# salesforce/warp-drive

Measured on AMD Instinct MI355X. Metric: env steps/sec, TagContinuous 5 taggers x 100 runners, higher is better.
Workload: dtype f32; 1 GPU; BASELINE configs[2]: TagContinuous 5 taggers x 100 runners, partial obs K=10 (F=71), num_envs=2000 per GPU; tick = sample_actions (2 heads) + step + reset of finished replicas (one fused launch); num_envs_per_gpu=2000, num_agents=105, launch_mode=plan, kernels_per_tick=1, ticks_per_launch=1, parallelism=env-replica sharding x1

## Files before the change

warp_drive_amd/csrc/kernels/tc_fast.h:

```cpp
#pragma once
#include "wd_common.h"
#include "tc_fetch.h"
#include "tc_sample.h"
#include "tc_move.h"
#include "tc_tags.h"
#include "tc_reset.h"
#include "tc_knn.h"
#include "tc_rows.h"

namespace {

template <int KMAX, bool FUSED, bool EXACTK, int IDB, bool SAMPLE = FUSED, bool LOOP = false, int SN = 0, int SA = 0,
          int ST = 0>
__device__ __forceinline__ int tc_fast_impl(const TcArgs &a, const TcFuse &fz, unsigned char *smem, int n_acc,
                                            int n_turn, int tick = 0, int n_taggers_in = 0, TcCarry *cy = nullptr,
                                            const TcLoopConsts *lc = nullptr) {
  WD_TC_PROBE_TICK(LOOP, tick);
  const int N = a.N, K = EXACTK ? KMAX : a.K;
  const int F = 7 * K + 1;
  int tid_ = threadIdx.x;
  if constexpr (LOOP) asm volatile("" : "+v"(tid_));
  const int tid = tid_, T_ = WD_TC_BLOCKDIM;
  const int epb = max(1, T_ / N);
  const int n_waves = (T_ + 63) >> 6, wave = __builtin_amdgcn_readfirstlane(tid >> 6), lane = tid & 63;
  const size_t slab_acc_bytes = tc_align16((size_t)4 * epb * N * n_acc);
  const bool compact = (epb == 1);
  const size_t slab_turn_bytes = tc_align16((size_t)4 * epb * N * n_turn);
  const bool one_slab = tc_one_slab(N);
  const TcFastLds l = tc_carve_fast(smem, epb, N, K, n_waves,
                                    !SAMPLE ? 0 : one_slab ? max(slab_acc_bytes, slab_turn_bytes) : slab_acc_bytes + slab_turn_bytes,
                                    compact);
  const TcTables &tb = l.tb;
  float *const slab_acc = (float *)smem, *const slab_turn = (float *)(smem + (one_slab ? 0 : slab_acc_bytes));
  float *const stage = l.stage + (size_t)wave * l.stage_dwords;
  const int el = tid / N, ag = tid - el * N;
  const float invK = 1.0f / (float)K, invN = 1.0f / (float)N;
  const int NP = ((N + 3) & ~3) + 8;

  int group = blockIdx.x;
#ifndef WD_TC_BLOCK_ORDER_PLAIN
  if constexpr (IDB == 7) {
    const int bx = blockIdx.x & 7, bq = gridDim.x >> 3, br = gridDim.x & 7;
    group = bx * bq + min(bx, br) + (int)(blockIdx.x >> 3);
  }
#endif
  const int env0 = a.env_begin + group * epb;
  __builtin_amdgcn_s_setprio(3);
  WD_TC_PROBE_RT(16); WD_TC_PROBE(0); WD_TC_PROBE_HW(21);
  TcIn in;
  bool reloaded = false;
  if constexpr (LOOP) {
    in = cy->in;
    reloaded = cy->reload != 0;
    if (reloaded) {
      tc_load_state(in, a, fz, env0, epb, N, n_acc, n_turn, tid, tick == 0);
      cy->in.type = in.type; cy->in.skill = in.skill; cy->in.step_reward = in.step_reward;
    }
  } else {
    tc_issue_loads<FUSED, SAMPLE>(in, a, fz, env0, epb, N, n_acc, n_turn, tid, slab_acc, slab_turn, true);
  }
  const bool tab_in_lds = (n_acc <= WD_TC_TAB) && (n_turn <= WD_TC_TAB);
  int n_taggers_ = n_taggers_in;
  if constexpr (LOOP) {
    if (tick == 0) n_taggers_ = tc_build_tables(tb, a, N, n_acc, n_turn, tab_in_lds, in);
  } else {
    n_taggers_ = tc_build_tables(tb, a, N, n_acc, n_turn, tab_in_lds, in);
  }
  const int n_taggers = n_taggers_;
  if (env0 >= a.E) return n_taggers;
  if constexpr (!LOOP) WD_TC_PROBE(1);

  const int env = env0 + el;
  const bool active = (el < epb) && (env < a.E);
  const int gi = env * N + ag;
  const int li = tid;
  const int agents_here = min(epb, a.E - env0) * N;
  if constexpr (LOOP) {
    if (active && ag == 0) a.done[env] = 0;
    static_assert(!LOOP || (SN > 0 && SA > 0 && ST == WD_TC_BLOCKDIM), "the multi-tick entry is built for one shape");
    tc_fetch_slabs_straight<SN, SA, ST>(slab_acc, slab_turn, fz.probs_acc, fz.probs_turn, env0, wave, lane);
    WD_TC_PROBE(1);
  }
  int2 sampled = in.sampled;
  const unsigned long long live_mask = __ballot(active && in.sg != 0);
  if constexpr (!LOOP) {
    if (compact && lane == 0) tb.live_cnt[wave] = __popcll(live_mask);
  }
  if constexpr ((IDB != 7) && (KMAX <= 12)) {
    if (compact && tid < 64) tb.cell_cnt[tid] = 0;
  }
  if constexpr (LOOP) {
    static_assert(!LOOP || IDB == 7, "tc_sample_heads_carried samples from two slabs: replicas of at most 128 agents");
    sampled = tc_sample_heads_carried<SA>(fz, in.epoch, cy->k0, cy->k1, active, gi, li, slab_acc, slab_turn, n_acc, n_turn);
    if (compact && lane == 0) tb.live_cnt[wave] = __popcll(live_mask);
  } else if (FUSED) {
    if (active && ag == 0) a.done[env] = 0;
    if (SAMPLE) sampled = tc_sample_heads(a, fz, in, active, gi, li, slab_acc, slab_turn, n_acc, n_turn, env0, epb);
  }
  WD_TC_PROBE(2);
  __syncthreads();
  WD_TC_PROBE(3);
  int my_c = ag, n_live = N;
  if (compact) {
    int before = 0;
    n_live = 0;
    for (int w2 = 0; w2 < n_waves; ++w2) {
      const int c = tb.live_cnt[w2];
      before += (w2 < wave) ? c : 0;
      n_live += c;
    }
    my_c = before + __popcll(live_mask & ((1ull << lane) - 1ull));
  }
  constexpr bool PRE = (IDB != 7) && (KMAX <= 12);
  constexpr bool TIE_TABLE = (IDB != 7);
  bool pre_on = false;
  int cells_C = 0;
  float cell_len = 0.0f, cell_inv = 0.0f;
  int my_cell = 0, my_cell_slot = 0;
  uint4 hint_a = make_uint4(~0u, ~0u, ~0u, ~0u), hint_b = hint_a;
  if constexpr (PRE) {
    pre_on = compact && (a.knn_prev != nullptr) && (n_live >= WD_TC_PRE_MIN_LIVE) && (l.stage_dwords >= WD_TC_LIST_DWORDS);
    if (pre_on && active && in.sg != 0) {
      const uint4 *const h = (const uint4 *)(a.knn_prev + (size_t)(env * N + ag) * 8);
      hint_a = h[0];
      hint_b = h[1];
    }
    if (pre_on) {
      cells_C = tc_cell_grid(n_live, K);
      cell_len = a.grid_length / (float)max(cells_C, 1);
      cell_inv = (float)cells_C / a.grid_length;
    }
  }

  float edge_pen = 0.0f, my_x = 0.0f, my_y = 0.0f;
  const int sg = in.sg;
  const bool is_runner = active && (in.type == 0) && (sg != 0);
  if (active) {
    const TcMoved m = tc_move<LOOP>(a, tb, in, sampled, gi, tab_in_lds, LOOP ? cy : nullptr, LOOP ? lc : nullptr);
    edge_pen = m.edge_pen; my_x = m.x; my_y = m.y;
    if constexpr (LOOP) {
      cy->in.x = m.x; cy->in.y = m.y;
      cy->in.cleared = (sg == 0) ? 1 : 0;
    }
    l.xy[el * NP + ag] = make_float2(sg ? m.x : (PRE && pre_on ? __builtin_nanf("") : WD_BIG), m.y);
    if (compact) {
      if (sg) {
        bool by_cell = false;
        if constexpr (PRE) {
          if (cells_C != 0) {
            const int2 c = tc_cell_xy(m.x, m.y, cell_inv, cells_C);
            my_cell = tc_cell_place(c, cells_C);
            my_cell_slot = atomicAdd(&tb.cell_cnt[my_cell], 1);
            by_cell = true;
          }
        }
        if (!by_cell) {
          l.xyc[my_c] = make_float2(m.x, m.y);
          l.cid[1 + my_c] = (short)ag;
          if (PRE && pre_on) {
            uint4 *const slot = (uint4 *)(l.stage + (size_t)(my_c >> 6) * l.stage_dwords) + 2 * (my_c & 63);
            slot[0] = hint_a;
            slot[1] = hint_b;
          }
        }
      }
      if (ag == 0) {
        l.cid[0] = -1;
        if (PRE && pre_on) {
          l.xyc[n_live] = make_float2(WD_BIG, WD_BIG);
          l.xy[N] = make_float2(__builtin_nanf(""), 0.0f);
        }
      }
    }
    tc_feat_store(l.feat, li, m.ft);
    l.sig[li] = (sg ? 1 : 0) | (in.cleared ? 2 : 0);
    if ((in.cleared != 0) != (sg == 0)) a.obs_rows_cleared[gi] = sg ? 0 : 1;
    l.tagcnt[li] = 0;
    if (ag == 0) {
      const int t = in.tstep + 1;
      a.timestep[env] = t;
      tb.tstep[el] = t;
      if constexpr (LOOP) tb.tfrac[el] = (float)tc_div_const((double)t, (double)a.T, lc->r_T);
      else tb.tfrac[el] = (float)((double)t / (double)a.T);
      if constexpr (LOOP) {
        cy->in.tstep = t;
        if (reloaded) tb.nrun[el] = in.nrun;
      } else {
        tb.nrun[el] = in.nrun;
      }
    }
  }
  WD_TC_PROBE(4);
  __syncthreads();
  WD_TC_PROBE(5);
  int cell_incl = 0;
  if constexpr (PRE) {
    if (cells_C != 0) {
      const int cnt = tb.cell_cnt[lane];
      cell_incl = cnt;
#pragma unroll
      for (int d = 1; d < 64; d <<= 1) {
        const int up = __shfl_up(cell_incl, d, 64);
        cell_incl += (lane >= d) ? up : 0;
      }
      my_c = __builtin_amdgcn_ds_bpermute(my_cell << 2, cell_incl - cnt) + my_cell_slot;
      if (active && sg != 0) {
        l.xyc[my_c] = make_float2(my_x, my_y);
        l.cid[1 + my_c] = (short)ag;
        uint4 *const slot = (uint4 *)(l.stage + (size_t)(my_c >> 6) * l.stage_dwords) + 2 * (my_c & 63);
        slot[0] = hint_a;
        slot[1] = hint_b;
      }
    }
  }

  bool tagged = false;
  if constexpr (LOOP) {
    if (is_runner)
      tagged = tc_find_tag<true>(a, tb, l.xy + el * NP, l.tagcnt + el * N, &tb.nrun[el], n_taggers, my_x, my_y, lc->Bc);
  } else {
    if (is_runner)
      tagged = tc_find_tag(a, tb, l.xy + el * NP, l.tagcnt + el * N, &tb.nrun[el], n_taggers, my_x, my_y);
  }
  if constexpr (PRE) {
    if (cells_C != 0) __syncthreads();
  }

  WD_TC_PROBE(6);
  int nid[KMAX + 1], rank[KMAX + 1];
#pragma unroll
  for (int k = 0; k <= KMAX; ++k) { nid[k] = -1; rank[k] = k; }
  bool in_order = true;
  __builtin_amdgcn_s_setprio(2);
  const bool searcher = compact ? (tid < n_live) : (active && sg != 0);
  const float2 *const sxy = compact ? l.xyc : l.xy + el * NP;
  const int n_cand = compact ? n_live : N;
  int row_agent = ag;
  constexpr int L = KMAX + ((EXACTK && IDB == 7) ? 2 : 3);
  const bool split = compact && (n_waves == 2) && (n_live <= 64) && (n_live >= 16) &&
                     (l.stage_dwords >= 64 * L);
  const int j_half = split ? (((n_live + 7) >> 3) << 2) : n_cand;
  const bool helper = split && (wave == 1);
  unsigned S[L];
  bool prefiltered = false;
  unsigned extra = 0xffffffffu;
  if constexpr (PRE) {
    if (pre_on) {
      unsigned Tb = 0u;
      float sx = 0.0f, sy = 0.0f;
      int2 scell = make_int2(0, 0);
      if (searcher) {
        const uint4 *const slot = (const uint4 *)stage + 2 * lane;
        const uint4 pa = slot[0], pb = slot[1];
        sx = sxy[ag].x; sy = sxy[ag].y;
        Tb = tc_knn_bound16<KMAX>(l.xy, N, sx, sy, pa, pb, K);
        if (cells_C != 0) {
          scell = tc_cell_xy(sx, sy, cell_inv, cells_C);
          Tb = min(Tb, tc_cell_cover2(sx, sy, scell, cell_len, cells_C));
        }
      }
      WD_TC_PROBE(7);
      if (__ballot(searcher) != 0ull && __ballot(searcher && Tb == 0x7f800000u) == 0ull) {
        const float Tf = searcher ? __uint_as_float(Tb) : -1.0f;
#pragma unroll
        for (int k = 0; k < L; ++k) S[k] = 0xffffffffu;
        const int C = cells_C;
        int r = 0, r_end = -1, run0 = 0, run1 = n_cand, x_lo = 0, y_lo = 0, x_hi = 0, y_hi = 0;
        if (C != 0) {
          const int last = min(63, __builtin_amdgcn_readfirstlane(n_live) - 1 - 64 * wave);
          x_lo = __builtin_amdgcn_readfirstlane(scell.x); y_lo = __builtin_amdgcn_readfirstlane(scell.y);
          x_hi = __builtin_amdgcn_readlane(scell.x, last); y_hi = __builtin_amdgcn_readlane(scell.y, last);
          r = max(0, y_lo - 1);
          r_end = min(C - 1, y_hi + 1);
          run1 = 0;
        }
        const TcPreList pl = tc_pre_list(stage, lane);
        int j = 0, j_end = 0;
        int listed = 0, words = 0;
        int probe_trips = 0;
        bool finished = false;
        while (!finished) {
          while (words < WD_TC_LIST_CAP) {
            if (j >= j_end) {
              bool flush = false;
              int p0 = 0, p1 = 0;
              while (!flush && r <= r_end) {
                int lo = C, hi = -1;
                for (int yy = max(y_lo, r - 1); yy <= min(y_hi, r + 1); ++yy) {
                  const bool fwd = (yy & 1) == 0;
                  const int from = (yy == y_lo) ? x_lo : (fwd ? 0 : C - 1), to = (yy == y_hi) ? x_hi : (fwd ? C - 1 : 0);
                  lo = min(lo, min(from, to));
                  hi = max(hi, max(from, to));
                }
                lo = max(0, lo - 1);
                hi = min(C - 1, hi + 1);
                const int first_cell = r * C + ((r & 1) ? C - 1 - hi : lo), last_cell = r * C + ((r & 1) ? C - 1 - lo : hi);
                ++r;
                if (hi < lo) continue;
                const int b = first_cell == 0 ? 0 : __builtin_amdgcn_readlane(cell_incl, max(first_cell, 1) - 1);
                const int e = __builtin_amdgcn_readlane(cell_incl, last_cell);
                const int j0 = max(run1, b & ~3), j1 = min(n_cand, (e + 3) & ~3);
                if (j1 <= j0) continue;
                if (run1 > run0 && j0 != run1) { p0 = run0; p1 = run1; flush = true; run0 = j0; run1 = j1; }
                else if (run1 > run0) run1 = j1;
                else { run0 = j0; run1 = j1; }
              }
              if (!flush) {
                if (run1 <= run0) { finished = true; break; }
                p0 = run0; p1 = run1; run0 = run1;
              }
              j = p0;
              j_end = p1;
            }
            const int j_stop = min(j_end, j + 32 * (WD_TC_LIST_CAP - words));
            tc_pre_pass1(sxy, sx, sy, j, j_stop, Tf, pl, listed);
            words += (j_stop - j + 31) >> 5;
            j = j_stop;
          }
          if (words != 0) tc_pre_pass2<L, IDB>(sxy, sx, sy, pl, listed, S, extra, probe_trips);
          listed = 0;
          words = 0;
        }
        WD_TC_PROBE_VAL(18, probe_trips);
        unsigned sK = S[KMAX];
#pragma unroll
        for (int k = 1; k < KMAX; ++k) sK = (k == K) ? S[k] : sK;
        const bool held = (sK >> IDB) + 2u <= (Tb >> IDB);
        prefiltered = __ballot(searcher && !held) == 0ull;
        WD_TC_PROBE_VAL(19, prefiltered ? 1 : 2);
        if (!prefiltered) extra = 0xffffffffu;
      }
      WD_TC_PROBE(8);
    }
  }
  if (!prefiltered && (searcher || (helper && lane < n_live))) {
    const int me = helper ? lane : ag;
    tc_chain_range<L, IDB>(sxy, sxy[me].x, sxy[me].y, helper ? j_half : 0, helper ? n_cand : j_half, S);
  }
  WD_TC_PROBE(9);
  if (split) {
    if (helper && lane < n_live) {
#pragma unroll
      for (int k = 0; k < L; ++k) ((unsigned *)stage)[64 * k + lane] = S[k];
      __builtin_amdgcn_s_setprio(0);
    }
    __syncthreads();
    if (searcher) {
      const unsigned *const theirs = (const unsigned *)(l.stage + (size_t)l.stage_dwords);
      unsigned P[L];
#pragma unroll
      for (int k = 0; k < L; ++k) P[k] = theirs[64 * k + lane];
      tc_merge_sorted<L>(S, P);
    }
  }
  bool exact = true;
  unsigned zone_hi = 0u;
  if (searcher) {
    unsigned o[L - 1];
    __builtin_amdgcn_s_setprio(1);
    exact = tc_resolve_keys<KMAX, IDB, L, TIE_TABLE>(sxy, ag, K, S, o, nid, rank, in_order, l.cid);
    WD_TC_PROBE(10);
    {
      unsigned oKth = o[KMAX - 1];
#pragma unroll
      for (int k = 0; k < KMAX - 1; ++k) oKth = (k == K - 1) ? o[k] : oKth;
      zone_hi = (oKth >> IDB) + 1u;
    }
    if constexpr (PRE) {
      if (pre_on) {
        unsigned w[8];
#pragma unroll
        for (int q = 0; q < 8; ++q) {
          unsigned pair = 0u;
#pragma unroll
          for (int h = 0; h < 2; ++h) {
            const int k = 2 * q + h;
            const unsigned key = (k < L - 1) ? o[k < L - 1 ? k : 0] : (k == L - 1) ? extra : 0xffffffffu;
            const unsigned id = (key >= 0x7f800000u) ? 0xffffu : (unsigned)(unsigned short)l.cid[1 + (key & ((1u << IDB) - 1u))];
            pair |= id << (16 * h);
          }
          w[q] = pair;
        }
        uint4 *const h = (uint4 *)(a.knn_prev + (size_t)(env * N + l.cid[1 + ag]) * 8);
        h[0] = make_uint4(w[0], w[1], w[2], w[3]);
        h[1] = make_uint4(w[4], w[5], w[6], w[7]);
      }
    }
    if (!exact && !(EXACTK && IDB == 7) && (IDB == 7 || n_cand <= 128)) {
      WD_TC_PROBE_VAL(20, 1);
      int nid2[KMAX], rank2[KMAX];
#pragma unroll
      for (int k = 0; k < KMAX; ++k) { nid2[k] = -1; rank2[k] = k; }
      tc_knn_registers<KMAX>(sxy, ag, n_cand, K, nid2, rank2);
#pragma unroll
      for (int k = 0; k < KMAX; ++k) { nid[k] = nid2[k]; rank[k] = rank2[k]; }
      nid[KMAX] = -1;
      rank[KMAX] = KMAX;
      in_order = false;
      exact = true;
    }
  }
  if constexpr (IDB != 7 || EXACTK) {
    unsigned long long need = __ballot(searcher && !exact);
    if (need != 0ull) {
      WD_TC_PROBE_VAL(20, 1);
      unsigned long long unresolved = 0ull;
      const float mx = searcher ? sxy[ag].x : 0.0f, my = searcher ? sxy[ag].y : 0.0f;
      while (need != 0ull) {
        const int fl = __ffsll((long long)need) - 1;
        need &= need - 1ull;
        const float sx = __builtin_bit_cast(float, __builtin_amdgcn_readlane(__builtin_bit_cast(int, mx), fl));
        const float sy = __builtin_bit_cast(float, __builtin_amdgcn_readlane(__builtin_bit_cast(int, my), fl));
        const unsigned zh = (unsigned)__builtin_amdgcn_readlane((int)zone_hi, fl);
        const int self = __builtin_amdgcn_readlane(ag, fl);
        const float2 *const zxy = compact ? sxy : l.xy + __builtin_amdgcn_readlane(el, fl) * NP;
        const int cnt = tc_zone_resolve<TIE_TABLE>(zxy, n_cand, sx, sy, self, zh, IDB, K, (unsigned char *)stage, lane, l.cid);
        if (cnt > 64) {
          unresolved |= 1ull << fl;
        } else {
          const unsigned short *const out = (const unsigned short *)((const unsigned char *)stage + 128 + 512);
#pragma unroll
          for (int k = 0; k < KMAX; ++k) {
            const int v = (k < K) ? (int)out[k] : -1;
            if (lane == fl) { nid[k] = v; rank[k] = k; }
          }
          if (lane == fl) { nid[KMAX] = -1; rank[KMAX] = KMAX; in_order = false; }
        }
        asm volatile("" ::: "memory");
        __builtin_amdgcn_wave_barrier();
      }
      if ((unresolved >> lane) & 1ull) {
        int nid2[KMAX];
#pragma unroll
        for (int k = 0; k < KMAX; ++k) nid2[k] = -1;
        tc_knn_scan<KMAX, TIE_TABLE>(sxy, ag, n_cand, K, nid2, l.cid);
#pragma unroll
        for (int k = 0; k < KMAX; ++k) { nid[k] = nid2[k]; rank[k] = k; }
        nid[KMAX] = -1;
        rank[KMAX] = KMAX;
        in_order = false;
      }
    }
  }
  if (searcher && compact) {
    row_agent = l.cid[1 + ag];
#pragma unroll
    for (int k = 0; k <= KMAX; ++k) nid[k] = l.cid[1 + nid[k]];
  }
  __builtin_amdgcn_s_setprio(0);
  WD_TC_PROBE(11);

  if constexpr (LOOP) {
    static_assert(!LOOP || (EXACTK && KMAX == 10 && IDB == 7), "the id rows of the multi-tick entry are built for K = 10");
    const bool any_out_of_order = __ballot(!in_order) != 0ull;
    if (searcher) {
      unsigned *const idrow = (unsigned *)(l.ids + row_agent * KMAX);
#pragma unroll
      for (int k = 0; k < KMAX; k += 2) idrow[k >> 1] = ((unsigned)nid[k] & 0xffffu) | ((unsigned)nid[k + 1] << 16);
      if (any_out_of_order && !in_order) {
        unsigned short *const hrow = l.ids + row_agent * KMAX;
#pragma unroll
        for (int k = 0; k <= KMAX; ++k)
          if (rank[k] < KMAX) hrow[rank[k]] = (unsigned short)(nid[k] < 0 ? 0xffff : nid[k]);
#pragma unroll
        for (int k = 0; k < KMAX; ++k) nid[k] = (int)((const short *)hrow)[k];
      }
      tc_store_id_row<false>(a.nearest_ids + (long)env0 * (SN * KMAX), __umul24((unsigned)row_agent, 4u * KMAX), nid);
    }
    if (active && sg == 0 && (reloaded || in.cleared == 0)) {
      int none[KMAX];
#pragma unroll
      for (int k = 0; k < KMAX; ++k) none[k] = -1;
      tc_store_id_row<true>(a.nearest_ids + (long)env0 * (SN * KMAX), __umul24((unsigned)ag, 4u * KMAX), none);
    }
  } else {
    const int ebase = el * N;
    const bool any_out_of_order = __ballot(!in_order) != 0ull;
    if (active && sg == 0) {
      unsigned short *const own = l.ids + (size_t)li * K;
#pragma unroll
      for (int k = 0; k < KMAX; ++k)
        if (k < K) own[k] = 0xffff;
    }
    if (searcher) {
      unsigned short *const idrow = l.ids + (size_t)(ebase + row_agent) * K;
#pragma unroll
      for (int k = 0; k < KMAX; ++k)
        if (k < K) idrow[k] = (unsigned short)(ebase + nid[k]);
      if (any_out_of_order && !in_order) {
#pragma unroll
        for (int k = 0; k <= KMAX; ++k)
          if (rank[k] < K) idrow[rank[k]] = (unsigned short)(nid[k] < 0 ? 0xffff : ebase + nid[k]);
      }
    }
  }
  __syncthreads();
  const int rpw = (agents_here + n_waves - 1) / n_waves;
  const int wrow0 = wave * rpw;
  const int wrows = max(0, min(rpw, agents_here - wrow0));
  if constexpr (!LOOP)
    tc_flush_ids(l.ids + (size_t)wrow0 * K, a.nearest_ids + ((long)env0 * N + wrow0) * K, wrows * K, lane, wrow0, N,
                 invK, invN, epb == 1);
  WD_TC_PROBE(12);
  const unsigned long long live_rows = __ballot(lane < wrows && (l.sig[wrow0 + lane] & 1));
  const int n_live_rows = __popcll(live_rows);
  constexpr int SPARSE_NUM = LOOP ? WD_TC_LOOP_SPARSE_NUM : 9, SPARSE_DEN = 16;
  if (n_live_rows * SPARSE_DEN <= wrows * SPARSE_NUM) {
    if constexpr (LOOP) {
      static_assert(!LOOP || (EXACTK && KMAX == 10), "the descriptor flush of the multi-tick entry is built for K = 10");
      tc_gather_rows_sparse<true, KMAX>(a, l, tb, stage, env0, wrow0, wrows, lane, K, N, invK, invN);
    } else {
      tc_gather_rows_sparse(a, l, tb, stage, env0, wrow0, wrows, lane, K, N, invK, invN);
    }
  } else if constexpr (LOOP) {
    static_assert(!LOOP || (EXACTK && KMAX == 10 && IDB == 7 && SN > 64 && SN <= 128), "two wavefronts, one replica per block");
    tc_gather_rows_dense_lean<KMAX, SN>(a, l, tb, stage, env0, wave, lane, live_rows);
  } else {
    int R = tc_stage_rows(F, n_waves);
    if constexpr (IDB != 7) {
      R = max(R, min(min(64, (l.stage_dwords - 20) / F), 192 / K));
    }
    constexpr int U = 3;
    int rr[U], so[U];
#pragma unroll
    for (int u = 0; u < U; ++u) {
      const int t = lane + 64 * u;
      rr[u] = (int)(((float)t + 0.5f) * invK);
      so[u] = rr[u] * F + (t - rr[u] * K);
    }
    float *const obs_w = a.obs + ((long)env0 * N + wrow0) * F;
    for (int r0 = 0; r0 < wrows; r0 += R) {
      const int rc = min(R, wrows - r0);
      float *const dst = obs_w + (long)r0 * F;
      const int mis = (int)(((size_t)dst >> 2) & 3);
      const int items = rc * K;
      const unsigned short *const idp = l.ids + (size_t)(wrow0 + r0) * K;
      const int fp = wrow0 + r0;
      int tt[U];
      unsigned jq[U];
#pragma unroll
      for (int u = 0; u < U; ++u) { tt[u] = min(lane + 64 * u, items - 1); jq[u] = idp[tt[u]]; }
      const bool clamped2 = lane + 128 >= items, clamped1 = lane + 64 >= items, clamped0 = lane >= items;
      TcFeat me[U], nb[U];
      int off[U];
#pragma unroll
      for (int u = 0; u < U; ++u) {
        const bool cl = (u == 0) ? clamped0 : (u == 1) ? clamped1 : clamped2;
        const int r_last = rc - 1, o_last = r_last * F + (K - 1);
        const int r = cl ? r_last : rr[u];
        off[u] = cl ? o_last : so[u];
        me[u] = tc_feat_load(l.feat, fp + r);
        const bool valid = ((me[u].type_sig & 1) != 0) && (jq[u] != 0xffffu);
        nb[u] = tc_feat_load(l.feat, valid ? (int)jq[u] : fp + r);
      }
#pragma unroll
      for (int u = 0; u < U; ++u) {
        const bool valid = ((me[u].type_sig & 1) != 0) && (jq[u] != 0xffffu);
        unsigned mv = valid ? 0xffffffffu : 0u;
        asm volatile("" : "+v"(mv));
        const unsigned ts = (unsigned)nb[u].type_sig & mv;
        float *o = stage + mis + off[u];
        o[0] = (float)(nb[u].nx - me[u].nx);
        o[K] = (float)(nb[u].ny - me[u].ny);
        o[2 * K] = nb[u].nsp - me[u].nsp;
        o[3 * K] = nb[u].nac - me[u].nac;
        o[4 * K] = nb[u].ndir - me[u].ndir;
        o[5 * K] = __uint_as_float(ts & 0x3f800000u);
        o[6 * K] = __uint_as_float((0u - (ts & 1u)) & 0x3f800000u);
      }
      if (lane < rc) {
        const int m = wrow0 + r0 + lane;
        const int e_m = (int)(((float)m + 0.5f) * invN);
        stage[mis + lane * F + 7 * K] = (l.sig[m] & 1) ? tb.tfrac[e_m] : 0.0f;
      }
      asm volatile("" ::: "memory");
      __builtin_amdgcn_wave_barrier();
      tc_flush_run(stage, dst, rc * F, lane);
      asm volatile("" ::: "memory");
      __builtin_amdgcn_wave_barrier();
    }
  }
  WD_TC_PROBE(13);
  __syncthreads();
  WD_TC_PROBE(14);

  if (active) tc_finish_agent(a, tb, el, ag, gi, env, sg, is_runner, tagged, l.tagcnt[li], edge_pen, in.step_reward, FUSED);
  if (FUSED) {
    __syncthreads();
    bool any = false;
    for (int e = 0; e < min(epb, a.E - env0); ++e) any = any || (tb.doneflag[e] != 0);
    if constexpr (LOOP) {
      if (active) {
        cy->in.sg = (tagged && a.runner_exits) ? 0 : sg;
        cy->in.epoch = in.epoch + 1u;
      }
      cy->reload = __builtin_amdgcn_readfirstlane(any ? 1 : 0);
    }
    if (any) {
      asm volatile("s_waitcnt vmcnt(0)" ::: "memory");
      __syncthreads();
      tc_reset_finished(a, fz, tb, env0, epb);
      if constexpr (LOOP) {
        asm volatile("s_waitcnt vmcnt(0)" ::: "memory");
        __syncthreads();
      }
    }
  }
  WD_TC_PROBE(15); WD_TC_PROBE_RT(17);
  return n_taggers;
}

template <int KMAX, bool EXACTK, int IDB, int SN, int SA, int ST>
__device__ __forceinline__ void tc_fast_rollout(const TcArgs &a, const TcFuse &fz, unsigned char *smem, int n_acc,
                                                int n_turn, int ticks) {
  int n_taggers = 0;
  TcCarry cy;
  cy.in = TcIn{};
  cy.reload = 1;
  cy.k0 = __builtin_amdgcn_readfirstlane(fz.rng_state[0]);
  cy.k1 = __builtin_amdgcn_readfirstlane(fz.rng_state[1]);
  const TcLoopConsts lc = tc_loop_consts(a.max_speed, a.grid_length, a.T, a.margin);
  for (int tick = 0; tick < ticks; ++tick) {
    n_taggers = tc_fast_impl<KMAX, true, EXACTK, IDB, true, true, SN, SA, ST>(a, fz, smem, n_acc, n_turn, tick, n_taggers, &cy,
                                                                              &lc);
    asm volatile("s_waitcnt vmcnt(0)" ::: "memory");
    __syncthreads();
  }
}

}
```

warp_drive_amd/csrc/kernels/tc_knn.h:

```cpp
#pragma once
#include "wd_common.h"
#include "tc_types.h"

namespace {


template <bool TABLE>
__device__ __forceinline__ int tc_tie_order(const short *tie, int idx) {
  if constexpr (TABLE) return tie ? (int)tie[1 + idx] : idx;
  else return idx;
}

struct TcP4 {
  float2 p[4];
};
__device__ __forceinline__ TcP4 tc_load4(const float2 *cxy, int j) {
  const float4 *const q = (const float4 *)__builtin_assume_aligned(cxy + j, 16);
  const float4 a = q[0], b = q[1];
  TcP4 r;
  r.p[0] = make_float2(a.x, a.y); r.p[1] = make_float2(a.z, a.w);
  r.p[2] = make_float2(b.x, b.y); r.p[3] = make_float2(b.z, b.w);
  return r;
}

template <int KMAX>
__device__ __forceinline__ void tc_rank_entries(const unsigned (&sb)[KMAX], int (&rank)[KMAX]) {
#pragma unroll
  for (int k = 0; k < KMAX; ++k) rank[k] = k;
#pragma unroll
  for (int i = 0; i < KMAX; ++i)
#pragma unroll
    for (int j = i + 1; j < KMAX; ++j) {
      const int c = (sb[j] < sb[i]) ? 1 : 0;
      rank[i] += c;
      rank[j] -= c;
    }
}

template <int KMAX>
__device__ __forceinline__ void tc_knn_registers(const float2 *cxy, int ag, int N, int K, int (&nid)[KMAX],
                                                 int (&rank)[KMAX]) {
  const float xi = cxy[ag].x, yi = cxy[ag].y;
  const float INF = __builtin_inff();

  float B[KMAX + 1];
#pragma unroll
  for (int k = 0; k <= KMAX; ++k) B[k] = INF;
#define WD_TC_INSERT(d2v)                                                                         \
  do {                                                                                            \
    _Pragma("unroll") for (int k = KMAX; k >= 1; --k) B[k] = __builtin_amdgcn_fmed3f(B[k - 1], B[k], (d2v)); \
    B[0] = fminf(B[0], (d2v));                                                                    \
  } while (0)
  {
    const int ng = N >> 2;
    TcP4 nxt = tc_load4(cxy, 0);
    for (int g = 0; g < ng; ++g) {
      const TcP4 cur = nxt;
      nxt = tc_load4(cxy, 4 * g + 4);
#pragma unroll
      for (int u = 0; u < 4; ++u) {
        const float dx = xi - cur.p[u].x, dy = yi - cur.p[u].y;
        const float d2 = dx * dx + dy * dy;
        WD_TC_INSERT(d2);
      }
    }
    for (int j = 4 * ng; j < N; ++j) {
      const float2 pj = cxy[j];
      const float dx = xi - pj.x, dy = yi - pj.y;
      const float d2 = dx * dx + dy * dy;
      WD_TC_INSERT(d2);
    }
  }
#undef WD_TC_INSERT
  __builtin_amdgcn_s_setprio(1);
  float T2 = INF;
#pragma unroll
  for (int k = 1; k <= KMAX; ++k) T2 = (k == K) ? B[k] : T2;
  float T2lo, T2hi;
  if (T2 == INF) {
    T2lo = INF; T2hi = 3.0e38f;
  } else if (T2 == 0.0f) {
    T2lo = 0.0f; T2hi = 0.0f;
  } else {
    const float S = sqrtf(T2);
    const float Sup = __uint_as_float(__float_as_uint(S) + 1u), Sdn = __uint_as_float(__float_as_uint(S) - 1u);
    const double mhi = 0.5 * ((double)S + (double)Sup), mlo = 0.5 * ((double)S + (double)Sdn);
    const double hi2 = mhi * mhi, lo2 = mlo * mlo;
    float th = (float)hi2, tl = (float)lo2;
    if ((double)th > hi2) th = __uint_as_float(__float_as_uint(th) - 1u);
    if ((double)tl < lo2) tl = __uint_as_float(__float_as_uint(tl) + 1u);
    T2hi = th;
    T2lo = tl;
  }
  unsigned sel[4] = {0u, 0u, 0u, 0u};
  int n_upto = 0;
#define WD_TC_PUSH(m, d2v, thr, op) \
  asm("v_cmp_" op "_f32 vcc, %1, %2\n\tv_addc_co_u32 %0, vcc, %0, %0, vcc" : "+v"(m) : "v"(d2v), "v"(thr) : "vcc")
  {
#define WD_TC_PUSH4(m, g)                                                       \
  do {                                                                          \
    float d_[4];                                                                \
    _Pragma("unroll") for (int u = 0; u < 4; ++u) {                             \
      const float dx = xi - (g).p[u].x, dy = yi - (g).p[u].y;                   \
      d_[u] = dx * dx + dy * dy;                                                \
    }                                                                           \
    WD_TC_PUSH(m, d_[0], T2hi, "le"); WD_TC_PUSH(m, d_[1], T2hi, "le");         \
    WD_TC_PUSH(m, d_[2], T2hi, "le"); WD_TC_PUSH(m, d_[3], T2hi, "le");         \
  } while (0)
    int w_first = 0;
    if (N >= 96) {
      unsigned m3[3] = {0u, 0u, 0u};
#define WD_TC_PUSH12(g0, g1, g2)                                                  \
  do {                                                                            \
    float e_[3][4];                                                               \
    _Pragma("unroll") for (int u = 0; u < 4; ++u) {                               \
      const float ax = xi - (g0).p[u].x, ay = yi - (g0).p[u].y;                   \
      const float bx = xi - (g1).p[u].x, by = yi - (g1).p[u].y;                   \
      const float cx = xi - (g2).p[u].x, cy = yi - (g2).p[u].y;                   \
      e_[0][u] = ax * ax + ay * ay; e_[1][u] = bx * bx + by * by; e_[2][u] = cx * cx + cy * cy; \
    }                                                                             \
    _Pragma("unroll") for (int u = 0; u < 4; ++u) {                               \
      WD_TC_PUSH(m3[0], e_[0][u], T2hi, "le");                                    \
      WD_TC_PUSH(m3[1], e_[1][u], T2hi, "le");                                    \
      WD_TC_PUSH(m3[2], e_[2][u], T2hi, "le");                                    \
    }                                                                             \
  } while (0)
      TcP4 a0 = tc_load4(cxy, 0), a1 = tc_load4(cxy, 32), a2 = tc_load4(cxy, 64), b0, b1, b2;
      for (int b = 0; b < 32; b += 8) {
        b0 = tc_load4(cxy, b + 4); b1 = tc_load4(cxy, b + 36); b2 = tc_load4(cxy, b + 68);
        WD_TC_PUSH12(a0, a1, a2);
        a0 = tc_load4(cxy, b + 8); a1 = tc_load4(cxy, b + 40); a2 = tc_load4(cxy, b + 72);
        WD_TC_PUSH12(b0, b1, b2);
      }
#undef WD_TC_PUSH12
#pragma unroll
      for (int w = 0; w < 3; ++w) {
        const unsigned self_bit = ((ag >> 5) == w) ? (1u << (ag & 31)) : 0u;
        sel[w] = __brev(m3[w]) & ~self_bit;
        n_upto += __popc(sel[w]);
      }
      w_first = 3;
    }
    TcP4 ga = tc_load4(cxy, 32 * w_first), gb;
#pragma unroll
    for (int w = 0; w < 4; ++w) {
      const int j0 = 32 * w;
      if (w >= w_first && j0 < N) {
        const int nb = min(32, N - j0);
        unsigned mu = 0u;
        int b = 0;
        for (; b + 8 <= nb; b += 8) {
          gb = tc_load4(cxy, j0 + b + 4);
          WD_TC_PUSH4(mu, ga);
          ga = tc_load4(cxy, j0 + b + 8);
          WD_TC_PUSH4(mu, gb);
        }
        if (b + 4 <= nb) {
          gb = tc_load4(cxy, j0 + b + 4);
          WD_TC_PUSH4(mu, ga);
          ga = gb;
          b += 4;
        }
        for (; b < nb; ++b) {
          const float2 pj = cxy[j0 + b];
          const float dx = xi - pj.x, dy = yi - pj.y;
          const float d2 = dx * dx + dy * dy;
          WD_TC_PUSH(mu, d2, T2hi, "le");
        }
        const unsigned self_bit = ((ag >> 5) == w) ? (1u << (ag & 31)) : 0u;
        sel[w] = (__brev(mu) >> (32 - nb)) & ~self_bit;
        n_upto += __popc(sel[w]);
      }
    }
#undef WD_TC_PUSH4
  }
  if (n_upto > K) {
    unsigned lo[4] = {0u, 0u, 0u, 0u};
    int c_less = 0;
#pragma unroll
    for (int w = 0; w < 4; ++w) {
      const int j0 = 32 * w;
      if (j0 < N) {
        const int nb = min(32, N - j0);
        unsigned mb = 0u;
        for (int b = 0; b < nb; ++b) {
          const float2 pj = cxy[j0 + b];
          const float dx = xi - pj.x, dy = yi - pj.y;
          const float d2 = dx * dx + dy * dy;
          WD_TC_PUSH(mb, d2, T2lo, "lt");
        }
        lo[w] = (__brev(mb) >> (32 - nb)) & sel[w];
        c_less += __popc(lo[w]);
      }
    }
    int quota = K - c_less;
#pragma unroll
    for (int w = 0; w < 4; ++w) {
      unsigned tie = sel[w] & ~lo[w];
      const int have_t = __popc(tie);
      if (have_t > quota) {
        unsigned kept = 0u;
        for (int q = 0; q < quota; ++q) { const unsigned bit = tie & (0u - tie); kept |= bit; tie ^= bit; }
        tie = kept;
      }
      quota -= min(have_t, quota);
      sel[w] = lo[w] | tie;
    }
  }
#undef WD_TC_PUSH
  int jj[KMAX];
#pragma unroll
  for (int k = 0; k < KMAX; ++k) {
    const int which = sel[0] ? 0 : sel[1] ? 1 : sel[2] ? 2 : sel[3] ? 3 : 4;
    const unsigned cur = sel[0] ? sel[0] : sel[1] ? sel[1] : sel[2] ? sel[2] : sel[3];
    jj[k] = (which < 4) ? which * 32 + (__ffs(cur) - 1) : -1;
    const unsigned cleared = cur & (cur - 1u);
    sel[0] = (which == 0) ? cleared : sel[0];
    sel[1] = (which == 1) ? cleared : sel[1];
    sel[2] = (which == 2) ? cleared : sel[2];
    sel[3] = (which == 3) ? cleared : sel[3];
  }
  float2 pp[KMAX];
#pragma unroll
  for (int k = 0; k < KMAX; ++k) pp[k] = cxy[jj[k] < 0 ? ag : jj[k]];
  unsigned sb[KMAX];
#pragma unroll
  for (int k = 0; k < KMAX; ++k) {
    const float dx = xi - pp[k].x, dy = yi - pp[k].y;
    sb[k] = (jj[k] >= 0) ? __float_as_uint(sqrtf(dx * dx + dy * dy)) : 0x7f800000u;
    nid[k] = jj[k];
  }
  tc_rank_entries<KMAX>(sb, rank);
}

template <int KMAX, bool TABLE = false>
__device__ __forceinline__ void tc_knn_scan(const float2 *cxy, int ag, int N, int K, int (&nid)[KMAX],
                                            const short *tie = nullptr) {
  const float xi = cxy[ag].x, yi = cxy[ag].y;
  float pd = -1.0f;
  int pj = -1, pt = -1;
#pragma unroll 1
  for (int k = 0; k < K; ++k) {
    float best = __builtin_inff();
    int bj = -1, bt = 0x7fffffff;
    for (int j = 0; j < N; ++j) {
      const float2 pc = cxy[j];
      const float dx = xi - pc.x, dy = yi - pc.y;
      const float d = sqrtf(dx * dx + dy * dy);
      if constexpr (TABLE) {
        const int tj = tc_tie_order<true>(tie, j);
        const bool above = (d > pd) || (d == pd && tj > pt);
        if (j != ag && above && (d < best || (d == best && tj < bt))) { best = d; bj = j; bt = tj; }
      } else {
        const bool above = (d > pd) || (d == pd && j > pj);
        if (j != ag && above && d < best) { best = d; bj = j; }
      }
    }
#pragma unroll
    for (int q = 0; q < KMAX; ++q) nid[q] = (q == k) ? bj : nid[q];
    if (bj < 0) break;
    pd = best;
    pj = bj;
    pt = bt;
  }
}

__device__ __forceinline__ unsigned tc_umed3(unsigned a, unsigned b, unsigned c) {
  unsigned r;
  asm("v_med3_u32 %0, %1, %2, %3" : "=v"(r) : "v"(a), "v"(b), "v"(c));
  return r;
}

template <int L, int IDB>
__device__ __forceinline__ void tc_chain_range(const float2 *cxy, float xi, float yi, int j0, int j1, unsigned (&S)[L]) {
  constexpr unsigned IDM = (1u << IDB) - 1u;
#pragma unroll
  for (int k = 0; k < L; ++k) S[k] = 0xffffffffu;
#define WD_TC_INSERT_KEY(d2v, jv)                                                          \
  do {                                                                                     \
    const unsigned key_ = (__float_as_uint(d2v) & ~IDM) | (unsigned)(jv);                  \
    _Pragma("unroll") for (int k = L - 1; k >= 1; --k) S[k] = tc_umed3(S[k - 1], S[k], key_); \
    S[0] = min(S[0], key_);                                                                \
  } while (0)
  const int g0 = j0 >> 2, ng = j1 >> 2;
#define WD_TC_INSERT_GROUP(grp, gidx)                                  \
  _Pragma("unroll") for (int u = 0; u < 4; ++u) {                      \
    const float dx = xi - (grp).p[u].x, dy = yi - (grp).p[u].y;        \
    const float d2 = dx * dx + dy * dy;                                \
    WD_TC_INSERT_KEY(d2, 4 * (gidx) + u);                              \
  }
  const int g_mid = (g0 + ng) >> 1;
  TcP4 ga = tc_load4(cxy, 4 * g0), gb;
  int g = g0;
  for (; g + 2 <= ng; g += 2) {
    gb = tc_load4(cxy, 4 * g + 4);
    asm volatile("" ::: "memory");
    if (g >= g_mid && g < g_mid + 2) __builtin_amdgcn_s_setprio(0);
    WD_TC_INSERT_GROUP(ga, g);
    ga = tc_load4(cxy, 4 * g + 8);
    asm volatile("" ::: "memory");
    WD_TC_INSERT_GROUP(gb, g + 1);
  }
  if (g < ng) {
    if (g >= g_mid) __builtin_amdgcn_s_setprio(0);
    WD_TC_INSERT_GROUP(ga, g);
  }
#undef WD_TC_INSERT_GROUP
  for (int j = max(4 * ng, j0); j < j1; ++j) {
    const float2 pj = cxy[j];
    const float dx = xi - pj.x, dy = yi - pj.y;
    const float d2 = dx * dx + dy * dy;
    WD_TC_INSERT_KEY(d2, j);
  }
#undef WD_TC_INSERT_KEY
}

__device__ __forceinline__ void tc_cex(unsigned &a, unsigned &b) {
  const unsigned lo = min(a, b), hi = max(a, b);
  a = lo;
  b = hi;
}
template <int L>
__device__ __forceinline__ void tc_merge_sorted(unsigned (&S)[L], const unsigned (&P)[L]) {
  constexpr int W = (L <= 8) ? 8 : (L <= 16) ? 16 : (L <= 32) ? 32 : 64;
  unsigned c[W];
#pragma unroll
  for (int k = 0; k < W; ++k) {
    const int q = W - 1 - k;
    c[k] = (k < L && q < L) ? min(S[k], P[q]) : (k < L) ? S[k] : (q < L) ? P[q] : 0xffffffffu;
  }
#pragma unroll
  for (int stride = W / 2; stride >= 1; stride >>= 1)
#pragma unroll
    for (int k = 0; k < W; ++k)
      if ((k & stride) == 0) tc_cex(c[k], c[k + stride]);
#pragma unroll
  for (int k = 0; k < L; ++k) S[k] = c[k];
}

#define WD_TC_PRE_MIN_LIVE 200

template <int KMAX>
__device__ __forceinline__ unsigned tc_knn_bound16(const float2 *xy_by_id, int pad_id, float xi, float yi, uint4 pa, uint4 pb,
                                                   int K) {
  constexpr int M = KMAX + 3;
  static_assert(M <= 15, "the remembered neighbours are sixteen 16-bit ids per agent, K + 3 of them in use");
  float2 p0, p1, p2, p3, p4, p5, p6, p7, p8, p9, p10, p11, p12, p13, p14;
#define WD_TC_PREV_POS(k, vec, word) \
  if (k < M) p##k = xy_by_id[min((vec.word >> (16 * (k & 1))) & 0xffffu, (unsigned)pad_id)]
  WD_TC_PREV_POS(0, pa, x); WD_TC_PREV_POS(1, pa, x); WD_TC_PREV_POS(2, pa, y); WD_TC_PREV_POS(3, pa, y);
  WD_TC_PREV_POS(4, pa, z); WD_TC_PREV_POS(5, pa, z); WD_TC_PREV_POS(6, pa, w); WD_TC_PREV_POS(7, pa, w);
  WD_TC_PREV_POS(8, pb, x); WD_TC_PREV_POS(9, pb, x); WD_TC_PREV_POS(10, pb, y); WD_TC_PREV_POS(11, pb, y);
  WD_TC_PREV_POS(12, pb, z); WD_TC_PREV_POS(13, pb, z); WD_TC_PREV_POS(14, pb, w);
#undef WD_TC_PREV_POS
  float far = 0.0f, far2 = 0.0f, far3 = 0.0f;
  unsigned n = 0u;
#define WD_TC_PREV_DIST(k)                                                                                  \
  if (k < M) {                                                                                              \
    const float dx = xi - p##k.x, dy = yi - p##k.y;                                                         \
    const float d2 = dx * dx + dy * dy;                                                                     \
    const float dz = fmaxf(d2, 0.0f);  \
    far3 = __builtin_amdgcn_fmed3f(far2, far3, dz);                                                         \
    far2 = __builtin_amdgcn_fmed3f(far, far2, dz);                                                          \
    far = fmaxf(far, dz);                                                                                   \
    asm("v_cmp_o_f32 vcc, %1, %1\n\tv_addc_co_u32 %0, vcc, 0, %0, vcc" : "+v"(n) : "v"(d2) : "vcc");       \
  }
  WD_TC_PREV_DIST(0) WD_TC_PREV_DIST(1) WD_TC_PREV_DIST(2) WD_TC_PREV_DIST(3) WD_TC_PREV_DIST(4)
  WD_TC_PREV_DIST(5) WD_TC_PREV_DIST(6) WD_TC_PREV_DIST(7) WD_TC_PREV_DIST(8) WD_TC_PREV_DIST(9)
  WD_TC_PREV_DIST(10) WD_TC_PREV_DIST(11) WD_TC_PREV_DIST(12) WD_TC_PREV_DIST(13) WD_TC_PREV_DIST(14)
#undef WD_TC_PREV_DIST
  const float T = (n >= (unsigned)(K + 2)) ? 1.15f * far3 : far * (1.15f * (float)(K + 3)) * __builtin_amdgcn_rcpf((float)n);
  return (n >= 5u) ? __float_as_uint(T) : 0x7f800000u;
}

__device__ __forceinline__ int tc_cell_grid(int n_live, int K) {
  const int c = (int)sqrtf((float)n_live * (3.14159265f / (2.2f * 2.2f)) / (float)K);
  return c >= 4 ? min(c, 8) : 0;
}
__device__ __forceinline__ int2 tc_cell_xy(float x, float y, float inv, int C) {
  return make_int2(min(C - 1, (int)(x * inv)), min(C - 1, (int)(y * inv)));
}
__device__ __forceinline__ int tc_cell_place(int2 c, int C) { return c.y * C + ((c.y & 1) ? C - 1 - c.x : c.x); }
__device__ __forceinline__ unsigned tc_cell_cover2(float x, float y, int2 c, float len, int C) {
  float cover = __builtin_inff();
  if (c.x > 0) cover = fminf(cover, x - (float)(c.x - 1) * len);
  if (c.x < C - 1) cover = fminf(cover, (float)(c.x + 2) * len - x);
  if (c.y > 0) cover = fminf(cover, y - (float)(c.y - 1) * len);
  if (c.y < C - 1) cover = fminf(cover, (float)(c.y + 2) * len - y);
  cover = fmaxf(cover - len * (1.0f / 1024.0f), 0.0f);
  return __float_as_uint(cover * cover);
}

#define WD_TC_LIST_CAP 11
#define WD_TC_LIST_DWORDS ((WD_TC_LIST_CAP + 1) * (64 + 32))
struct TcPreList {
  unsigned *masks;
  unsigned short *tops;
};
__device__ __forceinline__ TcPreList tc_pre_list(float *stage, int lane) {
  TcPreList pl;
  pl.masks = (unsigned *)stage + lane;
  pl.tops = (unsigned short *)((unsigned *)stage + (WD_TC_LIST_CAP + 1) * 64) + lane;
  return pl;
}

__device__ __forceinline__ void tc_pre_pass1(const float2 *cxy, float xi, float yi, int j0, int j1, float Tf, const TcPreList &pl,
                                             int &cnt) {
#define WD_TC_MASK_PUSH(m, d2v) (m) = __builtin_amdgcn_alignbit((m), __float_as_uint(Tf - (d2v)), 31)
#define WD_TC_MASK_PUSH4(m, grp)                                       \
  do {                                                                 \
    float d_[4];                                                       \
    _Pragma("unroll") for (int u = 0; u < 4; ++u) {                    \
      const float dx = xi - (grp).p[u].x, dy = yi - (grp).p[u].y;      \
      d_[u] = dx * dx + dy * dy;                                       \
    }                                                                  \
    WD_TC_MASK_PUSH(m, d_[0]); WD_TC_MASK_PUSH(m, d_[1]);              \
    WD_TC_MASK_PUSH(m, d_[2]); WD_TC_MASK_PUSH(m, d_[3]);              \
  } while (0)
  TcP4 ga = tc_load4(cxy, j0), gb;
  for (int jw = j0; jw < j1; jw += 32) {
    const int nb = min(32, j1 - jw);
    unsigned mo = 0xffffffffu;
    int b = 0;
    for (; b + 8 <= nb; b += 8) {
      gb = tc_load4(cxy, jw + b + 4);
      WD_TC_MASK_PUSH4(mo, ga);
      ga = tc_load4(cxy, jw + b + 8);
      WD_TC_MASK_PUSH4(mo, gb);
    }
    if (b + 4 <= nb) {
      gb = tc_load4(cxy, jw + b + 4);
      WD_TC_MASK_PUSH4(mo, ga);
      ga = gb;
      b += 4;
    }
    for (; b < nb; ++b) {
      const float2 pj = cxy[jw + b];
      const float dx = xi - pj.x, dy = yi - pj.y;
      const float d2 = dx * dx + dy * dy;
      WD_TC_MASK_PUSH(mo, d2);
    }
    const unsigned mu = ~mo;
    pl.masks[cnt * 64] = mu;
    pl.tops[cnt * 64] = (unsigned short)(jw + nb - 1);
    cnt += (mu != 0u) ? 1 : 0;
  }
#undef WD_TC_MASK_PUSH4
#undef WD_TC_MASK_PUSH
}

template <int L, int IDB>
__device__ __forceinline__ void tc_pre_pass2(const float2 *cxy, float xi, float yi, const TcPreList &pl, int cnt,
                                             unsigned (&S)[L], unsigned &extra, int &probe_trips) {
  constexpr unsigned IDM = (1u << IDB) - 1u;
  unsigned cur = (cnt > 0) ? pl.masks[0] : 0u;
  int top = pl.tops[0], pos1 = 1;
#ifdef WD_TC_PROBES
  int my_trips = 0;
#endif
  while (cur != 0u) {
#ifdef WD_TC_PROBES
    ++my_trips;
#endif
    const unsigned idx = (unsigned)(top - (__ffs(cur) - 1));
    cur &= cur - 1u;
    const float2 pj = cxy[idx];
    if (cur == 0u && pos1 < cnt) {
      cur = pl.masks[pos1 * 64];
      top = pl.tops[pos1 * 64];
      ++pos1;
    }
    const float dx = xi - pj.x, dy = yi - pj.y;
    const float d2 = dx * dx + dy * dy;
    const unsigned key_ = (__float_as_uint(d2) & ~IDM) | idx;
    extra = tc_umed3(S[L - 1], extra, key_);
#pragma unroll
    for (int k = L - 1; k >= 1; --k) S[k] = tc_umed3(S[k - 1], S[k], key_);
    S[0] = min(S[0], key_);
  }
#ifdef WD_TC_PROBES
  for (int o = 32; o > 0; o >>= 1) my_trips = max(my_trips, __shfl_xor(my_trips, o, 64));
  probe_trips += my_trips;
#endif
}

template <bool TABLE = false>
__device__ __forceinline__ int tc_zone_resolve(const float2 *cxy, int n_cand, float sx, float sy, int self, unsigned zone_hi,
                                               int idb, int K, unsigned char *scratch, int lane, const short *tie = nullptr) {
  unsigned short *const zl = (unsigned short *)scratch;
  unsigned long long *const keys = (unsigned long long *)(scratch + 128);
  unsigned short *const out = (unsigned short *)(scratch + 128 + 512);
  int cnt = 0;
  for (int j0 = 0; j0 < n_cand; j0 += 64) {
    const int j = j0 + lane;
    bool in = false;
    if (j < n_cand) {
      const float2 pj = cxy[j];
      const float dx = sx - pj.x, dy = sy - pj.y;
      const float d2 = dx * dx + dy * dy;
      in = (j != self) && ((__float_as_uint(d2) >> idb) <= zone_hi);
    }
    const unsigned long long m = __ballot(in);
    const int at = cnt + __popcll(m & ((1ull << lane) - 1ull));
    if (in && at < 64) zl[at] = (unsigned short)j;
    cnt += __popcll(m);
  }
  if (cnt > 64) return cnt;
  asm volatile("" ::: "memory");
  __builtin_amdgcn_wave_barrier();
  unsigned long long mine = ~0ull;
  if (lane < cnt) {
    const int j = zl[lane];
    const float2 pj = cxy[j];
    const float dx = sx - pj.x, dy = sy - pj.y;
    mine = ((unsigned long long)__float_as_uint(sqrtf(dx * dx + dy * dy)) << 32) |
           (TABLE ? ((unsigned)tc_tie_order<TABLE>(tie, j) << 16) : 0u) | (unsigned)j;
    keys[lane] = mine;
  }
  asm volatile("" ::: "memory");
  __builtin_amdgcn_wave_barrier();
  int r = 0;
  for (int u = 0; u < cnt; ++u) r += (keys[u] < mine) ? 1 : 0;
  if (lane < cnt && r < K) out[r] = (unsigned short)(mine & 0xffffu);
  asm volatile("" ::: "memory");
  __builtin_amdgcn_wave_barrier();
  return cnt;
}

template <int KMAX, int IDB, int L, bool TABLE = false>
__device__ __forceinline__ bool tc_resolve_keys(const float2 *cxy, int ag, int K, const unsigned (&S)[L],
                                                unsigned (&o)[L - 1], int (&nid)[KMAX + 1], int (&rank)[KMAX + 1],
                                                bool &in_order, const short *tie = nullptr) {
  static_assert(L == KMAX + 3 || L == KMAX + 2, "self + K others + two look-ahead entries (one: K == KMAX only)");
  constexpr bool ONE_LOOK = (L == KMAX + 2);
  constexpr unsigned IDM = (1u << IDB) - 1u;
  const float xi = cxy[ag].x, yi = cxy[ag].y;
  unsigned sv[L];
#pragma unroll
  for (int k = 0; k < L; ++k) {
    sv[k] = S[k];
    asm volatile("" : "+v"(sv[k]));
  }
  if (__ballot(sv[0] != (unsigned)ag) == 0ull) {
#pragma unroll
    for (int k = 0; k < L - 1; ++k) o[k] = sv[k + 1];
  } else {
    bool after = false;
#pragma unroll
    for (int k = 0; k < L - 1; ++k) {
      after = after || (sv[k] == (unsigned)ag);
      o[k] = after ? sv[k + 1] : sv[k];
    }
  }
  unsigned gap = 0xffffffffu;
#pragma unroll
  for (int k = 0; k < KMAX; ++k)
    if (k < K) gap = min(gap, o[k + 1] - o[k]);
  unsigned oKth = o[KMAX - 1];
#pragma unroll
  for (int k = 0; k < KMAX - 1; ++k) oKth = (k == K - 1) ? o[k] : oKth;
  const bool apart = (gap >= 3u * (IDM + 1u) - 1u) && (oKth < 0x7f800000u);
#pragma unroll
  for (int k = 0; k < KMAX; ++k) {
    nid[k] = (k < K) ? (int)(o[k] & IDM) : -1;
    rank[k] = k;
  }
  nid[KMAX] = -1;
  rank[KMAX] = KMAX;
  bool exact = true;
  in_order = apart;
  bool simple = false;
  if (!apart && oKth < 0x7f800000u) {
    constexpr unsigned THR = 3u * (IDM + 1u) - 1u;
    unsigned cm = 0u;
#pragma unroll
    for (int k = 0; k <= (ONE_LOOK ? KMAX - 1 : KMAX); ++k)
      if (k <= K) cm |= ((o[k + 1] - o[k] < THR) ? 1u : 0u) << k;
    unsigned rel = cm & ((1u << K) - 1u);
    const bool look_close = ONE_LOOK ? true : ((cm >> K) & 1u) != 0u;
    simple = ((rel & (rel >> 1)) == 0u) && !(((rel >> (K - 1)) & 1u) != 0u && look_close);
    if (simple) {
      WD_TC_PROBE_VAL(23, 1);
      while (rel) {
        const int q = __ffs(rel) - 1;
        rel &= rel - 1u;
        unsigned ka = o[0], kb = o[1];
#pragma unroll
        for (int k = 1; k < KMAX; ++k) {
          ka = (q == k) ? o[k] : ka;
          kb = (q == k) ? o[k + 1] : kb;
        }
        const int ia = (int)(ka & IDM), ib = (int)(kb & IDM);
        const float2 pa = cxy[ia], pb = cxy[ib];
        const float ax = xi - pa.x, ay = yi - pa.y, bx = xi - pb.x, by = yi - pb.y;
        const unsigned sa = __float_as_uint(sqrtf(ax * ax + ay * ay)), sb = __float_as_uint(sqrtf(bx * bx + by * by));
        if (sb < sa || (sb == sa && tc_tie_order<TABLE>(tie, ib) < tc_tie_order<TABLE>(tie, ia))) {
#pragma unroll
          for (int k = 0; k < KMAX; ++k) nid[k] = (k == q) ? ib : (k == q + 1 && k < K) ? ia : nid[k];
        }
      }
      in_order = true;
    }
  }
  if (!apart && !simple) {
    WD_TC_PROBE_VAL(22, 1);
    unsigned oK = o[KMAX - 1], oExtra = o[KMAX], oLook = o[ONE_LOOK ? KMAX : KMAX + 1];
#pragma unroll
    for (int k = 0; k < KMAX - 1; ++k) {
      oK = (k == K - 1) ? o[k] : oK;
      oExtra = (k == K - 1) ? o[k + 1] : oExtra;
      if constexpr (!ONE_LOOK) oLook = (k == K - 1) ? o[k + 2] : oLook;
    }
    const unsigned INVALID = 0x7f800000u;
    const unsigned cut = (oK >> IDB) + 2u;
    exact = (oK >= INVALID) || ((oLook >> IDB) >= cut);
    float2 pp[KMAX];
#pragma unroll
    for (int k = 0; k < KMAX; ++k) {
      const bool valid = (k < K) && (o[k] < INVALID);
      nid[k] = valid ? (int)(o[k] & IDM) : -1;
      pp[k] = cxy[valid ? nid[k] : ag];
    }
    unsigned long long key64[KMAX];
#pragma unroll
    for (int k = 0; k < KMAX; ++k) {
      const float dx = xi - pp[k].x, dy = yi - pp[k].y;
      const unsigned sb = (nid[k] >= 0) ? __float_as_uint(sqrtf(dx * dx + dy * dy)) : 0x7f800000u;
      key64[k] = ((unsigned long long)sb << 32) | (unsigned)(nid[k] < 0 ? nid[k] : tc_tie_order<TABLE>(tie, nid[k]));
    }
#pragma unroll
    for (int k = 0; k < KMAX; ++k) rank[k] = k;
#pragma unroll
    for (int i = 0; i < KMAX; ++i)
#pragma unroll
      for (int j = i + 1; j < KMAX; ++j) {
        const int c = (key64[j] < key64[i]) ? 1 : 0;
        rank[i] += c;
        rank[j] -= c;
      }
    nid[KMAX] = -1;
    rank[KMAX] = KMAX;
    if (!ONE_LOOK && oK < INVALID && oExtra < INVALID && (oExtra >> IDB) < cut) {
      const int idE = (int)(oExtra & IDM);
      const float2 pe = cxy[idE];
      const float dx = xi - pe.x, dy = yi - pe.y;
      const unsigned long long keyE = ((unsigned long long)__float_as_uint(sqrtf(dx * dx + dy * dy)) << 32) |
                                      (unsigned)tc_tie_order<TABLE>(tie, idE);
      int rE = K;
#pragma unroll
      for (int i = 0; i < KMAX; ++i) {
        const int c = (i < K && keyE < key64[i]) ? 1 : 0;
        rank[i] += c;
        rE -= c;
      }
      nid[KMAX] = idE;
      rank[KMAX] = rE;
    }
  }
  return exact;
}

}
```

Baseline: 128.4 million env_steps/s.

## Split kNN candidate scan across wave halves for 65-96 live agents

```diff
diff --git a/warp_drive_amd/csrc/kernels/tc_fast.h b/warp_drive_amd/csrc/kernels/tc_fast.h
--- a/warp_drive_amd/csrc/kernels/tc_fast.h
+++ b/warp_drive_amd/csrc/kernels/tc_fast.h
@@ -170,6 +170,10 @@
           l.xyc[n_live] = make_float2(WD_BIG, WD_BIG);
           l.xy[N] = make_float2(__builtin_nanf(""), 0.0f);
         }
+      }
+      if constexpr (LOOP) {
+        if (tc_lane_halves(compact, n_waves, n_live) && ag < 8 && n_live + ag < 2 * tc_half_len(n_live))
+          l.xyc[n_live + ag] = make_float2(WD_BIG, WD_BIG);
       }
     }
     tc_feat_store(l.feat, li, m.ft);
@@ -333,12 +337,45 @@
       WD_TC_PROBE(8);
     }
   }
-  if (!prefiltered && (searcher || (helper && lane < n_live))) {
+  bool half_lane = false;
+  int half_up = 0;
+  if constexpr (LOOP) {
+    const bool halves = tc_lane_halves(compact, n_waves, n_live) && (wave == 1);
+    const int h_len = tc_half_len(n_live);
+    half_lane = halves && ((lane & 31) < n_live - 64);
+    half_up = (halves && lane >= 32) ? h_len : 0;
+    if (searcher || (helper && lane < n_live) || half_lane) {
+      const int me = helper ? lane : halves ? 64 + (lane & 31) : ag;
+      tc_chain_range<L, IDB>(sxy + half_up, sxy[me].x, sxy[me].y, helper ? j_half : 0,
+                             helper ? n_cand : halves ? h_len : j_half, S);
+    }
+  } else if (!prefiltered && (searcher || (helper && lane < n_live))) {
     const int me = helper ? lane : ag;
     tc_chain_range<L, IDB>(sxy, sxy[me].x, sxy[me].y, helper ? j_half : 0, helper ? n_cand : j_half, S);
   }
   WD_TC_PROBE(9);
-  if (split) {
+  if constexpr (LOOP) {
+    unsigned P[L];
+    bool merge = false;
+    if (split) {
+      if (helper && lane < n_live) {
+#pragma unroll
+        for (int k = 0; k < L; ++k) ((unsigned *)stage)[64 * k + lane] = S[k];
+        __builtin_amdgcn_s_setprio(0);
+      }
+      __syncthreads();
+      if (searcher) {
+        const unsigned *const theirs = (const unsigned *)(l.stage + (size_t)l.stage_dwords);
+#pragma unroll
+        for (int k = 0; k < L; ++k) P[k] = theirs[64 * k + lane];
+        merge = true;
+      }
+    } else if (half_lane) {
+      tc_swap_lane_halves<L>(S, P, (unsigned)half_up);
+      merge = true;
+    }
+    if (merge) tc_merge_sorted<L>(S, P);
+  } else if (split) {
     if (helper && lane < n_live) {
 #pragma unroll
       for (int k = 0; k < L; ++k) ((unsigned *)stage)[64 * k + lane] = S[k];
diff --git a/warp_drive_amd/csrc/kernels/tc_knn.h b/warp_drive_amd/csrc/kernels/tc_knn.h
--- a/warp_drive_amd/csrc/kernels/tc_knn.h
+++ b/warp_drive_amd/csrc/kernels/tc_knn.h
@@ -338,6 +338,21 @@
   for (int k = 0; k < L; ++k) S[k] = c[k];
 }
 
+__device__ __forceinline__ bool tc_lane_halves(bool compact, int n_waves, int n_live) {
+  return compact && (n_waves == 2) && (n_live > 64) && (n_live <= 96);
+}
+__device__ __forceinline__ int tc_half_len(int n_live) { return ((n_live + 7) >> 3) << 2; }
+template <int L>
+__device__ __forceinline__ void tc_swap_lane_halves(unsigned (&S)[L], unsigned (&P)[L], unsigned up) {
+#pragma unroll
+  for (int k = 0; k < L; ++k) {
+    const unsigned s = S[k] + up;
+    const auto r = __builtin_amdgcn_permlane32_swap(s, s, false, false);
+    S[k] = r[0];
+    P[k] = r[1];
+  }
+}
+
 #define WD_TC_PRE_MIN_LIVE 200
 
 template <int KMAX>
```

After: 130.7 million env_steps/s (median of 6 runs). +1.7%, better.
